# C-H-Chien/Trifocal_Pose_Estimation_using_Improved_GPUHC

Measured on AMD Instinct MI355X. Metric: HC paths/sec (312 tracks x RANSAC samples), higher is better.
Workload: dtype f32

## Files before the change

trifocal_pose_estimation_using_improved_gpuhc_amd/_abi.py:

```python
from __future__ import annotations

import ctypes as C
import os
from collections import namedtuple

import numpy as np

PKG_DIR = os.path.dirname(os.path.abspath(__file__))
LIB_PATH = os.environ.get("HC_TRIFOCAL_LIB") or os.path.join(PKG_DIR, "lib", "libhc_trifocal.so")

ABI_VERSION = 2

NUM_VARS, NUM_PARAMS, NUM_TRACKS = 30, 33, 312
NPP = NUM_PARAMS + 1
UNIFIED_INDEX_SIZE = 38880

HC_STATUS = {0: "HC_SUCCESS", 1: "HC_ERROR_INVALID_VALUE", 2: "HC_ERROR_WORKSPACE", 3: "HC_ERROR_LAUNCH",
             4: "HC_ERROR_DEVICE", 5: "HC_ERROR_TABLE"}


class HCError(RuntimeError):
    pass


# ... 253 lines not shown
P2C_SIGNATURES = (
    Sig("hc_trifocal_2op1p_30x30_track_p2c", _ST, (_TA, C.POINTER(hcP2cArgs), *_WS), True),
    Sig("hc_trifocal_p2c_eval_batched", _ST, (_i, _p, _p, _p, _p, _p, _p, _p, _p, _p, *_WS), True),
    Sig("hc_p2c_coefficients", _ST, (_i, _p, _p, _p, _p, _p), True),
)
P2C_DECLARED_SYMBOLS = tuple(s.name for s in P2C_SIGNATURES)

_RS = C.POINTER(hcRefineSettings)
REFINE_SIGNATURES = (
    Sig("hc_trifocal_pose_refine", _ST, (_p, _i, _p, _p, _RS, _p, _p, _p), True),
    Sig("hc_trifocal_pose_refine_grouped", _ST, (_i, _p, _p, _RS, _p, _p, _p), True),
)
REFINE_DECLARED_SYMBOLS = tuple(s.name for s in REFINE_SIGNATURES)

HC_TOPK_MAX = 32
TOPK_SIGNATURES = (
    Sig("hc_trifocal_pose_topk_joint", _ST, (_i, _p, _p, _i, _p, _p), True),
    Sig("hc_trifocal_pose_topk_joint_grouped", _ST, (_i, _p, _p, _i, _p, _i, _p, _p), True),
    Sig("hc_trifocal_pose_refine_topk", _ST, (_i, _p, _i, _p, _p, _RS, _p, _p, _p, _p, _p), True),
    Sig("hc_trifocal_pose_refine_topk_grouped", _ST, (_i, _p, _i, _p, _RS, _p, _p, _p, _p, _p), True),
    Sig("hc_pose_merge_topk", None, (_i, _i, _p, _p, _p), True),
)
TOPK_DECLARED_SYMBOLS = tuple(s.name for s in TOPK_SIGNATURES)

LU_SIGNATURES = (
    Sig("hc_lu_step_level", _i, (_i,), True),
    Sig("hc_cgesv_30x30_struct_batched", _ST, (_i, _p, _p, _p, _p), True),
    Sig("hc_cgesv_30x30_variant_batched", _ST, (_i, _i, _p, _p, _p, _p), True),
)
LU_VARIANTS = ("throughput", "throughput_twin", "abort", "abort_twin", "small", "small_twin", "archived",
               "archived_twin")
LU_DECLARED_SYMBOLS = tuple(s.name for s in LU_SIGNATURES)

EVAL_SIGNATURES = (
    Sig("hc_trifocal_eval_variant_batched", _ST, (_i, _u, _i, _p, _p, _p, _p, _p, _p, _p, _p, _p, _p, *_WS), True),
)
EVAL_VARIANTS = ("packed", "abs")
HC_EVAL_REDO = 1
EVAL_DECLARED_SYMBOLS = tuple(s.name for s in EVAL_SIGNATURES)

ADAPTIVE_SIGNATURES = (
    Sig("hc_ransac_need_table", _ST, (_i, C.c_double, _i, _i, _p), True),
)
ADAPTIVE_DECLARED_SYMBOLS = tuple(s.name for s in ADAPTIVE_SIGNATURES)

_lib = None


def lib() -> C.CDLL:
    global _lib
    if _lib is None:
        if not os.path.exists(LIB_PATH):
            raise HCError(f"native library missing: {LIB_PATH} (run `python -c 'import __graft_entry__ as g; g.build()'`)")
        import torch
        L = C.CDLL(LIB_PATH)
        for s in SIGNATURES + P2C_SIGNATURES + REFINE_SIGNATURES + TOPK_SIGNATURES + LU_SIGNATURES + \
                EVAL_SIGNATURES + ADAPTIVE_SIGNATURES:
            fn = getattr(L, s.name, None)
            if fn is None:
                if s.optional:
                    continue
                raise HCError(f"{LIB_PATH} does not export {s.name}")
            fn.restype, fn.argtypes = s.restype, list(s.argtypes)
        if L.hc_trifocal_abi_version() != ABI_VERSION:
            raise HCError(f"{LIB_PATH}: ABI {L.hc_trifocal_abi_version()}, this binding expects {ABI_VERSION}")
        _lib = L
    return _lib


def check(status: int, what: str) -> None:
    if status != 0:
        detail = lib().hc_last_error_string().decode(errors="replace")
        raise HCError(f"{what} failed: {HC_STATUS.get(status, status)} ({detail})")


def call(name: str, *args) -> None:
    fn = getattr(lib(), name, None)
    if fn is None:
        raise HCError(f"{LIB_PATH} does not export {name}")
    check(fn(*args), name)


def ptr(x):
    if x is None:
        return C.c_void_p()
    if hasattr(x, "data_ptr"):
        return C.c_void_p(x.data_ptr())
    if hasattr(x, "cuda_stream"):
        return C.c_void_p(x.cuda_stream)
    return x.ctypes.data_as(C.c_void_p)
# ... 35 lines not shown
```

trifocal_pose_estimation_using_improved_gpuhc_amd/csrc/hc_components.hpp:

```cpp
#pragma once

#include "hc_layout.hpp"

namespace hc {


__global__ void __launch_bounds__(WG_THREADS) k_cgesv(int n, const cf *__restrict__ A, const cf *__restrict__ B,
                                                      cf *__restrict__ X) {
    __shared__ LUBuf s_lu[2 * WAVES_PER_WG];
    __shared__ __attribute__((aligned(16))) cf s_scr[2 * WAVES_PER_WG][LU_SCRATCH_CF];
    const int lane = lane_id();
    const int r = lane & 31;
    const int sys = (blockIdx.x * WAVES_PER_WG + threadIdx.x / WAVE) * 2 + (lane >> 5);
    const bool ok = sys < n && r < NV;
    cf rA[NV];
    uint32_t pat = 0;
#pragma unroll
    for (int c = 0; c < NV; c++) {
        rA[c] = ok ? A[((size_t)sys * NV + r) * NV + c] : cmk(0.0f, 0.0f);
        if (rA[c].x != 0.0f || rA[c].y != 0.0f) pat |= 1u << c;
    }
    const cf rB = ok ? B[(size_t)sys * NV + r] : cmk(0.0f, 0.0f);
    LUBuf &LB = s_lu[(threadIdx.x / WAVE) * 2 + (lane >> 5)];
    cf *scr = s_scr[(threadIdx.x / WAVE) * 2 + (lane >> 5)];
    bool redo;
    cf x = lu_solve<false>(rA, rB, lane, pat, LB, scr, redo, __ballot(sys < n));
    if (__builtin_expect(redo, 0)) {
#pragma unroll
        for (int c = 0; c < NV; c++) rA[c] = ok ? A[((size_t)sys * NV + r) * NV + c] : cmk(0.0f, 0.0f);
        x = lu_solve<true>(rA, rB, lane, pat, LB, scr, redo);
    }
    if (ok) X[(size_t)sys * NV + r] = x;
}

__global__ void __launch_bounds__(WG_THREADS) k_cgesv_struct_check(int n, const cf *__restrict__ A,
                                                                   unsigned *__restrict__ bad) {
    const size_t i = (size_t)blockIdx.x * WG_THREADS + threadIdx.x;
    if (i >= (size_t)n * NV) return;
    const uint32_t pat = LU_STRUCT_PAT[i % NV];
    bool out = false;
    for (int c = 0; c < NV; c++) {
        const cf a = A[i * NV + c];
        if (!((pat >> c) & 1u) && (a.x != 0.0f || a.y != 0.0f)) out = true;
    }
    if (out) *bad = 1u;
}
template <int LAT, bool STRUCT, bool ENTCHK, bool FUSE>
__global__ void __launch_bounds__(WG_THREADS) k_cgesv_variant(int n, const cf *__restrict__ A,
                                                              const cf *__restrict__ B, cf *__restrict__ X) {
    __shared__ LUBuf s_lu[2 * WAVES_PER_WG];
    __shared__ __attribute__((aligned(16))) cf s_scr[2 * WAVES_PER_WG][FUSE ? LU_SCRATCH_FUSED_CF : LU_SCRATCH_CF];
    const int lane = lane_id();
    const int r = lane & 31;
    const int sys = (blockIdx.x * WAVES_PER_WG + threadIdx.x / WAVE) * 2 + (lane >> 5);
    const bool ok = sys < n && r < NV;
    cf rA[NV];
    uint32_t nz = 0;
    pf2 sq = {0.0f, 0.0f};
#pragma unroll
    for (int c = 0; c < NV; c++) {
        rA[c] = ok ? A[((size_t)sys * NV + r) * NV + c] : cmk(0.0f, 0.0f);
        if constexpr (!STRUCT) {
            if (rA[c].x != 0.0f || rA[c].y != 0.0f) nz |= 1u << c;
        }
        if constexpr (ENTCHK) {
            sq.x = __builtin_fmaf(rA[c].x, rA[c].x, sq.x);
            sq.y = __builtin_fmaf(rA[c].y, rA[c].y, sq.y);
        }
    }
    bool ent_bad = false;
    if constexpr (ENTCHK) ent_bad = __ballot(!(sq.x + sq.y < __builtin_inff())) != 0ull;
    const uint32_t pat = STRUCT ? (r < NV ? LU_STRUCT_PAT[r] : 0u) : nz;
    const cf rB = ok ? B[(size_t)sys * NV + r] : cmk(0.0f, 0.0f);
    LUBuf &LB = s_lu[(threadIdx.x / WAVE) * 2 + (lane >> 5)];
    cf *scr = s_scr[(threadIdx.x / WAVE) * 2 + (lane >> 5)];
    bool redo;
    cf x = lu_solve<false, LAT, STRUCT, ENTCHK, FUSE>(rA, rB, lane, pat, LB, scr, redo, __ballot(sys < n), ent_bad);
    if (__builtin_expect(redo, 0)) {
#pragma unroll
        for (int c = 0; c < NV; c++) rA[c] = ok ? A[((size_t)sys * NV + r) * NV + c] : cmk(0.0f, 0.0f);
        x = lu_solve<true>(rA, rB, lane, pat, LB, scr, redo);
    }
    if (ok) X[(size_t)sys * NV + r] = x;
}
// ... 165 lines not shown
```

trifocal_pose_estimation_using_improved_gpuhc_amd/csrc/hc_kernels.hip:

```cpp
#include "hc_layout.hpp"
#include "hc_prep.hpp"
#include "hc_components.hpp"
#include "hc_ring.hpp"
#include "hc_score.hpp"
#include "hc_track.hpp"
#include "hc_p2c.hpp"
#include "../../include/hc_trifocal_testing.h"
#include "../../include/p2c/hc_trifocal_p2c.h"
#include "../../include/lu/hc_lu_testing.h"
#include "../../include/eval/hc_eval_testing.h"
#include "../../include/adaptive/hc_trifocal_adaptive.h"

#include <atomic>
#include <climits>
#include <cstdlib>
#include <cstring>
#include <map>
#include <mutex>
#include <utility>

namespace hc {

thread_local hipError_t g_last_hip_error = hipSuccess;
static inline hcStatus launch_status(hcStatus on_fail) {
    const hipError_t e = hipGetLastError();
    if (e != hipSuccess) { g_last_hip_error = e; return on_fail; }
    return HC_SUCCESS;
}

static size_t ws_bytes_needed() { return (sizeof(Workspace) + 255) & ~(size_t)255; }
struct SliceLayout {
    size_t rq, ring, susp;
    size_t total;
    unsigned long long ring_cap;
    size_t susp_entry0, susp_entry1;
};
static SliceLayout slice_layout(long long paths, int max_steps) {
    if (paths < 0) paths = 0;
    if (max_steps < 0) max_steps = 0;
    SliceLayout a;
    a.ring_cap = ring_entries(paths, max_steps);
    const size_t ring_bytes = ((size_t)a.ring_cap * sizeof(unsigned long long) + 255) & ~(size_t)255;
// ... 505 lines not shown
    if ((hc::g_last_hip_error = hipIpcOpenMemHandle(&p, h, hipIpcMemLazyEnablePeerAccess)) != hipSuccess)
        return HC_ERROR_DEVICE;
    *flag = (uint32_t *)p;
    return HC_SUCCESS;
}

hcStatus hc_shared_flag_reset(uint32_t *flag, hcStream stream) {
    if (!flag) return HC_ERROR_INVALID_VALUE;
    if ((hc::g_last_hip_error = hipMemsetAsync(flag, 0, sizeof(uint32_t), (hipStream_t)stream)) != hipSuccess)
        return HC_ERROR_LAUNCH;
    return HC_SUCCESS;
}

hcStatus hc_shared_flag_close(uint32_t *flag, int opened) {
    if (!flag) return HC_ERROR_INVALID_VALUE;
    if (!opened) {
        std::lock_guard<std::mutex> g(hc::g_flag_mu);
        hc::g_flag_kind.erase(flag);
    }
    hc::g_last_hip_error = opened ? hipIpcCloseMemHandle(flag) : hipFree(flag);
    return hc::g_last_hip_error == hipSuccess ? HC_SUCCESS : HC_ERROR_DEVICE;
}

int hc_trifocal_abi_version(void) { return HC_TRIFOCAL_ABI_VERSION; }

unsigned hc_lu_struct_pattern(int row) { return row >= 0 && row < hc::NV ? hc::LU_STRUCT_PAT[row] : 0u; }
unsigned hc_lu_candidates(int step) { return step >= 0 && step < hc::NV ? hc::LU_BOUND.cand[step] : 0u; }
int hc_lu_search_span(int step) { return step >= 0 && step < hc::NV ? hc::lu_search_span(step) : -1; }
int hc_lu_step_level(int step) { return step >= 0 && step < hc::NV ? hc::LU_LEVELS.level[step] : -1; }
int hc_lu_group_class(int step, int group) {
    if (step < 0 || step >= hc::NV - 1 || group < 0 || group >= hc::LuChunks::count(step)) return -1;
    return hc::lu_group_class(step, group);
}

hcStatus hc_trifocal_ring_check_test(void *workspace, size_t workspace_bytes, unsigned head, unsigned tail,
                                     unsigned avail, hcStream stream) {
    const hc::SliceLayout area = hc::slice_layout(0, 0);
    if (!workspace || workspace_bytes < area.ring) return HC_ERROR_WORKSPACE;
    hipStream_t s = (hipStream_t)stream;
    unsigned *rq = (unsigned *)((char *)workspace + area.rq);
    const unsigned v[3] = {head, tail, avail};
    const int at[3] = {hc::RQ_HEAD, hc::RQ_TAIL, hc::RQ_AVAIL};
    (void)hipGetLastError();
    for (int i = 0; i < 3; i++)
        if ((hc::g_last_hip_error = hipMemcpyAsync(rq + at[i], &v[i], sizeof(unsigned), hipMemcpyHostToDevice, s)) !=
            hipSuccess)
            return HC_ERROR_LAUNCH;
    if ((hc::g_last_hip_error = hipStreamSynchronize(s)) != hipSuccess) return HC_ERROR_DEVICE;
    hipLaunchKernelGGL(hc::k_ring_check, dim3(1), dim3(64), 0, s, (hc::Workspace *)workspace, (const unsigned *)rq);
    return hc::launch_status(HC_ERROR_LAUNCH);
}

void hc_trifocal_set_ring_test(int delay_ticks) {
    hc::g_ring_test.store(delay_ticks > 0 ? (delay_ticks < HC_RING_TEST_MIN_TICKS ? HC_RING_TEST_MIN_TICKS : delay_ticks)
                                          : 0,
                          std::memory_order_relaxed);
}

void hc_trifocal_set_small_launch(int mode) {
    hc::g_small_launch.store(mode < 0 ? -1 : mode > 0 ? 1 : 0, std::memory_order_relaxed);
}

void hc_trifocal_set_retry_reuse(int on) { hc::g_retry_reuse.store(on ? 1 : 0, std::memory_order_relaxed); }

const char *hc_trifocal_version(void) {
    return "hc_trifocal gfx950 v10.11 (2 paths/wave, structurally sparse LDS-broadcast LU with lean pivot steps fused by level, "
           "one exec region per pivot step for the eligible rows with the column groups through scratch windows, "
           "column groups by structural class (never-fillable groups untested, always-live groups unconditional), "
           "pivot search narrowed to the candidate rows' DPP group "
           "(abort kernel and tracking launches filling at most half of the path slots -- the latter at 3 waves/SIMD, "
           "16 columns per batch: batched latency mode, one LDS round trip per pivot step, every live-able column "
           "group untested), "
           "structure-agnostic twin kernels for other dH/dx structures, readlane back substitution (the throughput "
           "kernel's fused positions level by level through LDS), pipelined evals over "
           "per-slot prefix tables, 5 waves/SIMD, time slicing at step boundaries with least-attained-service "
           "issue priority, a rejected step's retry reuses its first RK4 slope, the throughput kernel's operand "
           "addresses read complete from per-slot tables and its finiteness check made on the dH/dx entries)";
}

}
```

trifocal_pose_estimation_using_improved_gpuhc_amd/csrc/hc_lu.hpp:

```cpp
#pragma once

#include "hc_eval.hpp"
#include "hc_lu_struct.hpp"
#include "hc_lu_diag.hpp"

namespace hc {

typedef float f4v __attribute__((ext_vector_type(4)));

struct alignas(16) LUBuf {
    cf row[32];
};
static_assert(sizeof(LUBuf) == sizeof(SlotLDS::lu), "LUBuf is SlotLDS::lu");
static_assert(offsetof(SlotLDS, lu) % 16 == 0, "SlotLDS::lu must be 16-B aligned");

__device__ __forceinline__ float rcp_rn(float s) {
    const float r0 = __builtin_amdgcn_rcpf(s);
    const float e0 = __builtin_fmaf(-s, r0, 1.0f);
    return __builtin_fmaf(e0, r0, r0);
}
__device__ __forceinline__ bool rcp_fast_bits(int bits) {
    return (uint32_t)(bits - 0x12800000) < (uint32_t)(0x7B800000 - 0x12800000);
}

// ... 388 lines not shown
            pl1 = 32 + __builtin_ctz((unsigned)(pm >> 32) | 0x80000000u);
            if constexpr (!DENSE)
                redo = redo || __builtin_amdgcn_ballot_w64(!rcp_fast_bits(__float_as_int(piv_abs))) != 0ull;
        } else if constexpr (TIE) {
            const int c2 = key == mx ? rowid : (1 << 20);
            const int mn = half_min_int_p16(c2);
            is_piv = key == mx && rowid == mn;
            piv_abs = __int_as_float(mx);
            const unsigned long long w = __builtin_amdgcn_ballot_w64(is_piv);
            piv_m = w;
            pl0 = __builtin_ctz((unsigned)w);
            pl1 = 32 + __builtin_ctz((unsigned)(w >> 32));
        } else {
            is_piv = __builtin_amdgcn_inverse_ballot_w64(m);
            piv_m = m;
            piv_abs = __int_as_float(mx);
            pl0 = __builtin_ctz(mlo);
            pl1 = 32 + __builtin_ctz(mhi);
        }
        HC_ISA_MARK_I("lu_pattern", I);
        if constexpr (DENSE) lu_step_dense<I>(rA, rB, rowid, my, L, is_piv, reg_s, oo_s, elig HC_LU_WORK_PASS);
        else if constexpr (LAT > 0 && STRUCT) lu_step_batched<I, LAT>(rA, rB, rowid, my, L, scr, is_piv, reg_s, oo_s, elig);
        else lu_step_tested<I, (LAT > 0), STRUCT>(rA, rB, rowid, pat, my, L, scr, is_piv, pl0, pl1, reg_s, oo_s,
                                                  elig HC_LU_WORK_PASS);
        lu_forward<I + 1, DENSE, LAT, STRUCT>(rA, rB, rowid, pat, lane, r, hb, row_lane, my, L, scr, redo,
                                              elig_m & ~piv_m HC_LU_WORK_PASS);
    }
}
template <int LV>
__device__ __forceinline__ void lu_forward_fused(cf (&rA)[NV], cf &rB, int &rowid, uint32_t &pat, int lane, int r, int hb,
                                                 bool row_lane, PivF &my, LUBuf &L, cf *scr, bool &redo,
                                                 unsigned long long elig_m HC_LU_WORK_ARG) {
    if constexpr (LV < LU_LEVELS.nlevels) {
        if (!lu_level<LV>(rA, rB, rowid, pat, lane, r, hb, my, scr, elig_m HC_LU_WORK_PASS)) {
#ifdef HC_DIAG_LUWORK
            lu_work_acc.rare++;
            lu_work_acc.rare_fusable = 1ull;
#endif
            redo = true;
            return;
        }
        lu_forward_fused<LV + 1>(rA, rB, rowid, pat, lane, r, hb, row_lane, my, L, scr, redo, elig_m HC_LU_WORK_PASS);
    } else {
        lu_forward<lu_first_unfused_step(), false, 0, true>(rA, rB, rowid, pat, lane, r, hb, row_lane, my, L, scr, redo,
                                                           elig_m HC_LU_WORK_PASS);
    }
}

template <int I, int LAST = 0>
__device__ __forceinline__ void lu_backward(const cf (&rA)[NV], cf &rB, int rowid, const PivF &my, pf2 &res) {
    if constexpr (I >= LAST) {
        HC_ISA_MARK_I("lu_back", I);
        const unsigned long long own = __builtin_amdgcn_ballot_w64(rowid == I);
        const int o0 = __builtin_ctz((unsigned)own);
        const int o1 = 32 + __builtin_ctz((unsigned)(own >> 32));
        const pf2 q = pcdiv_apply(pf2{rB.x, rB.y}, pf2{rA[I].x, rA[I].y}, my);
        const float x0 = __int_as_float(__builtin_amdgcn_readlane(__float_as_int(q.x), o0));
        const float y0 = __int_as_float(__builtin_amdgcn_readlane(__float_as_int(q.y), o0));
        const float x1 = __int_as_float(__builtin_amdgcn_readlane(__float_as_int(q.x), o1));
        const float y1 = __int_as_float(__builtin_amdgcn_readlane(__float_as_int(q.y), o1));
        const pf2 xs0 = {x0, y0}, xs1 = {x1, y1};
        pf2 xv;
        unsigned long long tmp;
        asm volatile("s_nop 1\n\ts_mov_b64 %2, exec\n\tv_mov_b64 %0, %3\n\ts_mov_b32 exec_lo, 0\n\t"
                     "v_mov_b64 %0, %4\n\ts_mov_b32 exec_lo, %5\n\ts_mov_b32 exec_hi, %5\n\t"
                     "v_mov_b64 %1, %0\n\ts_mov_b64 exec, %2"
                     : "=&v"(xv), "+v"(res), "=&s"(tmp) : "s"(xs0), "s"(xs1), "i"(1u << I));
// ... 10 lines not shown
    const bool entchk = !ABORT && !ARCH && LULAT == 0;
    return LuMode{LULAT, LUS, entchk, entchk && LUS};
}

template <bool DENSE, int LAT = 0, bool STRUCT = false, bool ENTCHK = false, bool FUSE = false>
__device__ __forceinline__ cf lu_solve(cf (&rA)[NV], cf rB, int lane, uint32_t pattern, LUBuf &L, cf *scratch,
                                      bool &redo, unsigned long long count_mask = ~0ull, bool ent_bad = false) {
    static_assert(!FUSE || (!DENSE && LAT == 0 && STRUCT && ENTCHK), "the fused levels belong to the throughput tracker's solve");
    (void)count_mask;
    const int r = lane & 31, hb = lane & 32;
    const bool row_lane = r < NV;
    redo = false;
    if constexpr (DENSE) HC_ISA_MARK("lu_dense");
    else HC_ISA_MARK("lu_sparse");
    HC_ISA_MARK("lu_finite");
    if constexpr (!DENSE && ENTCHK) {
        if (__builtin_expect(ent_bad, 0)) {
            redo = true;
            return cmk(0.0f, 0.0f);
        }
    } else if constexpr (!DENSE) {
        pf2 sq = {0.0f, 0.0f};
#pragma unroll
        for (int c = 0; c < NV; c++) {
            const pf2 e = {rA[c].x, rA[c].y};
            asm("v_pk_fma_f32 %0, %1, %1, %0" : "+v"(sq) : "v"(e));
        }
        const bool ok = sq.x + sq.y < __builtin_inff();
        if (__builtin_expect(__builtin_amdgcn_ballot_w64(!ok) != 0ull, 0)) {
            redo = true;
            return cmk(0.0f, 0.0f);
        }
    }
    int rowid = row_lane ? r : 99;
    uint32_t pat = row_lane ? pattern : 0u;
    PivF my{pf2{0.0f, 0.0f}};
#ifdef HC_DIAG_LUWORK
    LuWork lu_work_acc{0ull, count_mask, 0ull, 0ull, 0ull, 0ull};
#endif
    if constexpr (FUSE)
        lu_forward_fused<0>(rA, rB, rowid, pat, lane, r, hb, row_lane, my, L, scratch + 2 * r, redo,
                            __builtin_amdgcn_ballot_w64(row_lane) HC_LU_WORK_PASS);
    else
        lu_forward<0, DENSE, LAT, STRUCT>(rA, rB, rowid, pat, lane, r, hb, row_lane, my, L, scratch + 2 * r, redo,
                                          __builtin_amdgcn_ballot_w64(row_lane) HC_LU_WORK_PASS);
#ifdef HC_DIAG_LUWORK
    const unsigned long long solves = (unsigned long long)__builtin_popcountll(count_mask & __builtin_amdgcn_ballot_w64(row_lane)) / NV;
    if (lane == 0 && !DENSE && !redo) {
        atomicAdd(&g_diag_luwork[0], lu_work_acc.acc);
        atomicAdd(&g_diag_luwork[1], solves);
        atomicAdd(&g_diag_luwork[3], 1ull);
        atomicAdd(&g_diag_luwork[4], lu_work_acc.groups);
        atomicAdd(&g_diag_luwork[5], lu_work_acc.rare);
    }
    if (lane == 0 && DENSE) atomicAdd(&g_diag_luwork[2], solves);
    if (lane == 0 && !DENSE) atomicAdd(&g_diag_luwork[DIAG_LUWORK_RARE_FUSABLE], lu_work_acc.rare_fusable);
#endif
    if constexpr (FUSE) {
        if (__builtin_expect(redo, 0)) return cmk(0.0f, 0.0f);
    }
#ifdef HC_DIAG_PHASES
    if ((lane & 63) == 0 && blockIdx.x < 16384u) g_diag_lu_mid[blockIdx.x * 4 + (threadIdx.x >> 6)] = __builtin_amdgcn_s_memtime();
#endif
    HC_ISA_MARK("lu_back_init");
    pf2 res = {0.0f, 0.0f};
    if constexpr (FUSE) {
        lu_backward<NV - 1, lu_first_unfused_step()>(rA, rB, rowid, my, res);
// ... 20 lines not shown
```

trifocal_pose_estimation_using_improved_gpuhc_amd/csrc/hc_lu_levels.hpp:

```cpp
#pragma once

namespace hc {

constexpr int DPP_WAVE_SHL1 = 0x130, DPP_WAVE_SHR1 = 0x138;

template <int LV, int K>
__device__ __forceinline__ void lvl_pick(const cf (&rA)[NV], pf2 &c, uint32_t &bnd, int &cwo) {
    if constexpr (K < lu_level_count(LV)) {
        constexpr int I = lu_level_member(LV, K);
        const bool in = __builtin_amdgcn_inverse_ballot_w64(lu_both(LU_BOUND.cand[I]));
        c.x = in ? rA[I].x : c.x;
        c.y = in ? rA[I].y : c.y;
        bnd = in ? LU_BOUND.s[I] : bnd;
        cwo = in ? LU_CHAIN_WIN0 + 2 * K : cwo;
        lvl_pick<LV, K + 1>(rA, c, bnd, cwo);
    }
}
template <int LV, int K>
__device__ __forceinline__ void lvl_relabel(int &rowid, unsigned long long m, int hb) {
    if constexpr (K < lu_level_count(LV)) {
        constexpr int I = lu_level_member(LV, K);
        const unsigned long long mi = and_halves<LU_BOUND.cand[I]>(m);
        const int p0 = __builtin_amdgcn_readlane(rowid, __builtin_ctz((unsigned)mi));
        const int p1 = __builtin_amdgcn_readlane(rowid, 32 + __builtin_ctz((unsigned)(mi >> 32)));
        const int piv_pos = hb ? p1 : p0;
        const bool is_p = __builtin_amdgcn_inverse_ballot_w64(mi);
        rowid = is_p ? I : (rowid == I ? piv_pos : rowid);
        lvl_relabel<LV, K + 1>(rowid, m, hb);
    }
}
template <int LV, int J>
__device__ __forceinline__ void lvl_groups(cf (&rA)[NV], const pf2 &l, cf *wrow, const cf *cw) {
    if constexpr (J < NV) {
        if constexpr (((LU_LEVELS.cols[LV] >> J) & 3u) != 0u) {
            grp_store<J, 2>(wrow, rA);
            wave_lds_sync();
            cf u[2];
            grp_load<J, 2>(cw, u);
            grp_update<J, 2>(rA, l, u);
            __builtin_amdgcn_sched_barrier(0);
        }
        lvl_groups<LV, J + 2>(rA, l, wrow, cw);
    }
}
template <int LV>
__device__ __forceinline__ bool lu_level(cf (&rA)[NV], cf &rB, int &rowid, uint32_t &pat, int lane, int r, int hb,
                                         PivF &my, cf *scr, unsigned long long &elig_m HC_LU_WORK_ARG) {
    constexpr int CNT = lu_level_count(LV), I0 = lu_level_member(LV, 0);
    constexpr uint32_t ROWS = LU_LEVELS.rows[LV];
    HC_ISA_MARK_I("lu_search", I0);
    pf2 c = {0.0f, 0.0f};
    uint32_t bnd = 0u;
    int cwo = 0;
    lvl_pick<LV, 0>(rA, c, bnd, cwo);
    const float v = __builtin_fabsf(c.x) + __builtin_fabsf(c.y);
    pf2 oo_s;
    const pf2 reg_s = recip_fast(c, v, oo_s);
    const unsigned long long lv_elig = and_halves<ROWS>(elig_m);
    const bool elig = __builtin_amdgcn_inverse_ballot_w64(lv_elig);
    const int key = elig ? __float_as_int(v) : -1;
    int mx;
    {
        const int u1 = dpp_i<DPP_WAVE_SHL1>(key), u2 = dpp_i<DPP_WAVE_SHL1>(u1);
        const int d1 = dpp_i<DPP_WAVE_SHR1>(key), d2 = dpp_i<DPP_WAVE_SHR1>(d1);
        const int a = __builtin_amdgcn_inverse_ballot_w64(lu_both(LU_TRI0 | LU_TRI1)) ? u1 : -1;
        const int b = __builtin_amdgcn_inverse_ballot_w64(lu_both(LU_TRI0)) ? u2 : -1;
        const int e = __builtin_amdgcn_inverse_ballot_w64(lu_both(LU_TRI1 | LU_TRI2)) ? d1 : -1;
        const int f = __builtin_amdgcn_inverse_ballot_w64(lu_both(LU_TRI2)) ? d2 : -1;
        mx = max(max(key, a), max(b, max(e, f)));
    }
    constexpr uint32_t UP9 = lu_partner_rows(LV, 9), DN9 = lu_partner_rows(LV, -9), UP6 = lu_partner_rows(LV, 6),
                       DN6 = lu_partner_rows(LV, -6);
    static_assert((UP9 | DN9 | UP6 | DN6 | lu_partner_rows(LV, 0)) == (1u << NV) - 1u, "partner triples 6 or 9 lanes away");
    if constexpr ((UP9 | DN9 | UP6 | DN6) != 0u) {
        int pl = lane;
        if constexpr (UP9 != 0u) pl = __builtin_amdgcn_inverse_ballot_w64(lu_both(UP9)) ? lane + 9 : pl;
        if constexpr (DN9 != 0u) pl = __builtin_amdgcn_inverse_ballot_w64(lu_both(DN9)) ? lane - 9 : pl;
        if constexpr (UP6 != 0u) pl = __builtin_amdgcn_inverse_ballot_w64(lu_both(UP6)) ? lane + 6 : pl;
        if constexpr (DN6 != 0u) pl = __builtin_amdgcn_inverse_ballot_w64(lu_both(DN6)) ? lane - 6 : pl;
        mx = max(mx, __builtin_amdgcn_ds_bpermute(pl << 2, mx));
    }
    const unsigned long long m = and_halves<ROWS>(__builtin_amdgcn_ballot_w64(key == mx));
    const unsigned long long bad = and_halves<ROWS>(__builtin_amdgcn_ballot_w64(!rcp_fast_bits(mx)));
    if (__builtin_expect((__builtin_popcountll(m) != 2 * CNT) | (bad != 0ull), 0)) return false;
    const bool is_piv = __builtin_amdgcn_inverse_ballot_w64(m);
    HC_ISA_MARK_I("lu_store", I0);
    const cf *cw = scr + (cwo - 2 * r);
    cf *wrow = is_piv ? const_cast<cf *>(cw) : scr;
    st4(&wrow[0], cmk(reg_s.x, reg_s.y), rB);
    wave_lds_sync();
    HC_ISA_MARK_I("lu_rcp", I0);
    cf reg, sB0;
    ld4(&cw[0], reg, sB0);
    if (is_piv) my.oo = oo_s;
    asm volatile("" : "+v"(my.oo));
    lvl_relabel<LV, 0>(rowid, m, hb);
    HC_ISA_MARK_I("lu_update", I0);
#ifdef HC_DIAG_LUWORK
    {
        int pairs = 0;
        for (int j = 0; j < NV; j += 2) pairs += ((LU_LEVELS.cols[LV] >> j) & 3u) != 0u;
        lu_work_acc.acc += 2ull * (unsigned long long)pairs *
                           (unsigned long long)__builtin_popcountll(lv_elig & lu_work_acc.mask & ~m);
        lu_work_acc.groups += (unsigned long long)pairs;
    }
#endif
    if (elig) {
        HC_ISA_MARK_I("lu_mult", I0);
        const pf2 lq = pcmul(c, pf2{reg.x, reg.y});
        const pf2 lp = {is_piv ? 0.0f : lq.x, is_piv ? 0.0f : lq.y};
        const pf2 bp = pcmsub(pf2{rB.x, rB.y}, lp, pf2{sB0.x, sB0.y});
        rB = cmk(bp.x, bp.y);
        pat |= (pat & lu_member_cols(LV)) != 0u ? bnd : 0u;
        lvl_groups<LV, 0>(rA, lp, wrow, cw);
    }
    elig_m &= ~m;
    return true;
}

template <int LV, int K>
__device__ __forceinline__ void lvl_back_pick(const cf (&rA)[NV], pf2 &c, int &mem) {
    if constexpr (K < lu_level_count(LV)) {
        constexpr int I = lu_level_member(LV, K);
        if constexpr (K == 0) {
            c = pf2{rA[I].x, rA[I].y};
            mem = I;
        } else {
            const bool in = __builtin_amdgcn_inverse_ballot_w64(lu_both(LU_BOUND.cand[I]));
            c.x = in ? rA[I].x : c.x;
            c.y = in ? rA[I].y : c.y;
            mem = in ? I : mem;
        }
        lvl_back_pick<LV, K + 1>(rA, c, mem);
    }
}
template <int LV>
__device__ __forceinline__ void lu_back_level(const cf (&rA)[NV], cf &rB, int rowid, const PivF &my, LUBuf &L) {
    HC_ISA_MARK_I("lu_back_level", LV);
    pf2 c;
    int mem;
    lvl_back_pick<LV, 0>(rA, c, mem);
    const pf2 q = pcdiv_apply(pf2{rB.x, rB.y}, c, my);
    if (rowid == mem) L.row[mem] = cmk(q.x, q.y);
    wave_lds_sync();
    if constexpr (LV > 0) {
        if (__builtin_amdgcn_inverse_ballot_w64(lu_both(LU_LEVELS.rows[LV]))) {
            const cf x = L.row[mem];
            const pf2 w = pcmsub(pf2{rB.x, rB.y}, pf2{x.x, x.y}, c);
            rB = cmk(w.x, w.y);
        }
    }
}
template <int LV>
__device__ __forceinline__ void lu_backward_fused(const cf (&rA)[NV], cf &rB, int rowid, const PivF &my, LUBuf &L, int r,
                                                  pf2 &res) {
    if constexpr (LV >= 0) {
        lu_back_level<LV>(rA, rB, rowid, my, L);
        lu_backward_fused<LV - 1>(rA, rB, rowid, my, L, r, res);
    } else {
        if (__builtin_amdgcn_inverse_ballot_w64(lu_both(lu_fused_steps()))) {
            const cf x = L.row[r];
            res = pf2{x.x, x.y};
        }
    }
}

}
```

trifocal_pose_estimation_using_improved_gpuhc_amd/csrc/hc_lu_struct.hpp:

```cpp
#pragma once

#include <initializer_list>

#include "hc_device.hpp"

namespace hc {

constexpr int LU_CHUNK = 2;

struct LuChunks {
    static constexpr int single(int I) { return ((I + 1) & 1) && (I + 1 < NV) ? 1 : 0; }
    static constexpr int start(int I, int k) { return k < single(I) ? I + 1 : I + 1 + single(I) + (k - single(I)) * LU_CHUNK; }
    static constexpr int len(int I, int k) {
        return k < single(I) ? 1 : ((NV - start(I, k)) < LU_CHUNK ? (NV - start(I, k)) : LU_CHUNK);
    }
    static constexpr int count(int I) { return single(I) + (NV - (I + 1 + single(I)) + LU_CHUNK - 1) / LU_CHUNK; }
    static constexpr uint32_t mask(int I, int k) { return ((1u << len(I, k)) - 1u) << start(I, k); }
};

constexpr uint32_t LU_STRUCT_PAT[NV] = {
    0x7040004u, 0x7080004u, 0x7100004u, 0x7040009u, 0x7080009u, 0x7100009u, 0x7040012u, 0x7080012u,
    0x7100012u, 0x38200020u, 0x38400020u, 0x38800020u, 0x38200041u, 0x38400041u, 0x38800041u, 0x38200082u,
    0x38400082u, 0x38800082u, 0x7003100u, 0x7003100u, 0x7001100u, 0x7018400u, 0x7018400u, 0x7008400u,
    0x38005200u, 0x38005200u, 0x38001200u, 0x38028800u, 0x38028800u, 0x38008800u};
// ... 149 lines not shown
        if (!((c >> row) & 1u) || lu_popcount(c) <= 3) continue;
        int lo = 0, hi = 31;
        while (!((c >> lo) & 1u)) lo++;
        while (!((c >> hi) & 1u)) hi--;
        return row < lo + 3 ? (hi - 2) - lo : lo - (hi - 2);
    }
    return 0;
}
constexpr uint32_t lu_partner_rows(int lv, int off) {
    uint32_t m = 0u;
    for (int r = 0; r < NV; r++)
        if (lu_partner_off(lv, r) == off) m |= 1u << r;
    return m;
}
constexpr bool lu_chains_are_triples() {
    for (int i = 0; i < NV; i++) {
        if (!lu_step_fusable(i)) continue;
        uint32_t c = LU_BOUND.cand[i], t = 0u;
        for (int q = 0; q < NV; q += 3)
            if (((c >> q) & 7u) == 7u) t |= 7u << q;
        if (t != c) return false;
    }
    return true;
}
static_assert(lu_chains_are_triples(), "a fusable step's candidates are not whole lane triples");
constexpr uint32_t lu_member_cols(int lv) { return LU_LEVELS.fused[lv]; }
constexpr unsigned long long lu_both(uint32_t m) { return (unsigned long long)m | ((unsigned long long)m << 32); }
constexpr uint32_t LU_TRI0 = 0x09249249u, LU_TRI1 = LU_TRI0 << 1, LU_TRI2 = LU_TRI0 << 2;

constexpr int LU_SCRATCH_CF = 2 * 31 + 32;
constexpr int LU_CHAIN_WIN0 = LU_SCRATCH_CF;
constexpr int LU_SCRATCH_FUSED_CF = LU_CHAIN_WIN0 + 2 * (lu_max_level_count() - 1) + 32;

}
```

trifocal_pose_estimation_using_improved_gpuhc_amd/csrc/hc_track_body.inc:

```
    constexpr LuMode LUM = lu_mode(ABORT, ARCH, LULAT, LUS);
    constexpr bool LUSTRUCT = LUM.strct;
    constexpr bool ABSTAB = LUM.entchk;
    constexpr bool LUFUSE = LUM.fuse;
    __shared__ cf s_sp[NPP];
    __shared__ SlotLDS s_slot[2 * WAVES_PER_WG];
    Workspace *ws = a.ws;
    const EvalTables *T = &ws->tab;
    if (ws->status != 0u) return;
    if ((T->lu_struct == 1u) != LUSTRUCT) return;
    const unsigned epoch = (!ABORT && a.slice_q > 0) ? ld_rlx(&a.rq[RQ_EPOCH]) : 0u;
    const uint2 *s_ht = T->ht;
    const uint32_t *s_hx = T->hx;
    const uint32_t *s_hxd = &T->hxd[0][0];
    if (!P2C && threadIdx.x < NPP) s_sp[threadIdx.x] = a.start_params[threadIdx.x];
    {
        float *z = reinterpret_cast<float *>(s_slot);
        for (int i = threadIdx.x; i < (int)(sizeof(s_slot) / 4); i += WG_THREADS) z[i] = 0.0f;
    }
    __syncthreads();
    if (ABORT && threadIdx.x == 0) atomicCAS(&ws->t_start, 0ull, (unsigned long long)__builtin_amdgcn_s_memrealtime());
    const int lane = lane_id();
    const int r = lane & 31, hb = lane & 32;
    const int wid = threadIdx.x / WAVE;
    SlotLDS &S = s_slot[wid * 2 + (hb >> 5)];
    if (r == 30) S.x[30] = cmk(1.0f, 0.0f);
    if (r == 0) S.st.pre_smp = -2;
    __shared__ uint32_t s_rowc[GM_WORDS + 1][32];
    if (threadIdx.x < 32) {
        for (int q = 0; q < GM_WORDS; q++) s_rowc[q][threadIdx.x] = T->gm[q][threadIdx.x];
        s_rowc[GM_WORDS][threadIdx.x] = T->pat[threadIdx.x];
    }
    __syncthreads();
    const bool rl = r < NV;
    wave_lds_sync();
    const AbsTables *AT = &ws->abs;
    const int wv = ABSTAB ? __builtin_amdgcn_readfirstlane(wid) : 0;
    char *const l0 = reinterpret_cast<char *>(s_slot);

    int ph = PH_DEQ, b = -1, smp_loaded = -1;
    int qpos = 0;
    unsigned found_seen = 0u;
#ifdef HC_DIAG_TIMES
    int diag_t0 = 0;
    const unsigned long long diag_w0 = __builtin_amdgcn_s_memrealtime();
    if (lane == 0) atomicMin(&g_diag_span[0], diag_w0);
#endif
    int s = 0, stepidx = 0, coef = 1, succ = 0, nsteps = 0, ncorr = 0;
    int piece = 0;
    float t0 = 0.0f, t_step = 0.0f, dt = 0.01f, h2 = 0.0f, scale = 0.0f;
    bool end_zone = false, check = true, isSucc = false, isInf = false;
    cf x = cmk(0.0f, 0.0f), xl = x, sols = x;
    constexpr bool REUSE = !ABORT && !ARCH;
    bool k1v = false;

#ifdef HC_DIAG_PHASES
    uint64_t dg[8] = {0, 0, 0, 0, 0, 0, 0, 0};
    uint64_t dt_ = __builtin_amdgcn_s_memtime(), dt0_ = dt_;
#define HC_DIAG_MARK(k) do { const uint64_t n_ = __builtin_amdgcn_s_memtime(); dg[k] += n_ - dt_; dt_ = n_; } while (0)
#else
#define HC_DIAG_MARK(k) do { } while (0)
#endif
    for (;;) {
        HC_DIAG_MARK(6);
        HC_ISA_MARK("ctl_slots");
// ... 537 lines not shown
```

Measured before the change: 1.603 million.

## Read fused LU level row constants and row labels from LDS tables

Replaces the per-level chains of compile-time inverse-ballot selects (chain pick, bound, window offset, partner lane, triple-place masks) with a single packed per-row record word loaded from a small LDS table that each workgroup fills at kernel start. Row relabeling after a pivot level now goes through an LDS row-to-position map instead of per-member readlane sequences. The aim is to cut the scalar and VALU instruction count of each fused pivot level. In exchange it adds LDS reads, a table fill with a barrier, a loop in the relabel, and more LDS use that could reduce workgroups per CU.

```diff
diff --git a/include/lu/hc_lu_rowtable_testing.h b/include/lu/hc_lu_rowtable_testing.h
--- /dev/null
+++ b/include/lu/hc_lu_rowtable_testing.h
@@ -0,0 +1,23 @@
+#ifndef HC_LU_ROWTABLE_TESTING_H
+#define HC_LU_ROWTABLE_TESTING_H
+
+#ifdef __cplusplus
+extern "C" {
+#endif
+
+typedef enum {
+    HC_LU_ROW_MEMBER = 0,
+    HC_LU_ROW_BOUND = 1,
+    HC_LU_ROW_WINDOW = 2,
+    HC_LU_ROW_PARTNER = 3,
+    HC_LU_ROW_PLACE = 4,
+    HC_LU_ROW_CHAIN = 5,
+    HC_LU_ROW_FIELD_COUNT = 6
+} hcLuRowField;
+
+int hc_lu_row_field(int level, int row, int field);
+
+#ifdef __cplusplus
+}
+#endif
+#endif
diff --git a/trifocal_pose_estimation_using_improved_gpuhc_amd/_abi.py b/trifocal_pose_estimation_using_improved_gpuhc_amd/_abi.py
--- a/trifocal_pose_estimation_using_improved_gpuhc_amd/_abi.py
+++ b/trifocal_pose_estimation_using_improved_gpuhc_amd/_abi.py
@@ -309,6 +309,11 @@
                "archived_twin")
 LU_DECLARED_SYMBOLS = tuple(s.name for s in LU_SIGNATURES)
 
+LU_ROWTABLE_SIGNATURES = (
+    Sig("hc_lu_row_field", _i, (_i, _i, _i), True),
+)
+LU_ROW_FIELDS = ("member", "bound", "window", "partner", "place", "chain")
+
 EVAL_SIGNATURES = (
     Sig("hc_trifocal_eval_variant_batched", _ST, (_i, _u, _i, _p, _p, _p, _p, _p, _p, _p, _p, _p, _p, *_WS), True),
 )
@@ -332,7 +337,7 @@
         import torch
         L = C.CDLL(LIB_PATH)
         for s in SIGNATURES + P2C_SIGNATURES + REFINE_SIGNATURES + TOPK_SIGNATURES + LU_SIGNATURES + \
-                EVAL_SIGNATURES + ADAPTIVE_SIGNATURES:
+                LU_ROWTABLE_SIGNATURES + EVAL_SIGNATURES + ADAPTIVE_SIGNATURES:
             fn = getattr(L, s.name, None)
             if fn is None:
                 if s.optional:
diff --git a/trifocal_pose_estimation_using_improved_gpuhc_amd/csrc/hc_components.hpp b/trifocal_pose_estimation_using_improved_gpuhc_amd/csrc/hc_components.hpp
--- a/trifocal_pose_estimation_using_improved_gpuhc_amd/csrc/hc_components.hpp
+++ b/trifocal_pose_estimation_using_improved_gpuhc_amd/csrc/hc_components.hpp
@@ -50,6 +50,10 @@
                                                               const cf *__restrict__ B, cf *__restrict__ X) {
     __shared__ LUBuf s_lu[2 * WAVES_PER_WG];
     __shared__ __attribute__((aligned(16))) cf s_scr[2 * WAVES_PER_WG][FUSE ? LU_SCRATCH_FUSED_CF : LU_SCRATCH_CF];
+    if constexpr (FUSE) {
+        lu_rowtab_fill(threadIdx.x);
+        __syncthreads();
+    }
     const int lane = lane_id();
     const int r = lane & 31;
     const int sys = (blockIdx.x * WAVES_PER_WG + threadIdx.x / WAVE) * 2 + (lane >> 5);
diff --git a/trifocal_pose_estimation_using_improved_gpuhc_amd/csrc/hc_kernels.hip b/trifocal_pose_estimation_using_improved_gpuhc_amd/csrc/hc_kernels.hip
--- a/trifocal_pose_estimation_using_improved_gpuhc_amd/csrc/hc_kernels.hip
+++ b/trifocal_pose_estimation_using_improved_gpuhc_amd/csrc/hc_kernels.hip
@@ -8,6 +8,7 @@
 #include "../../include/hc_trifocal_testing.h"
 #include "../../include/p2c/hc_trifocal_p2c.h"
 #include "../../include/lu/hc_lu_testing.h"
+#include "../../include/lu/hc_lu_rowtable_testing.h"
 #include "../../include/eval/hc_eval_testing.h"
 #include "../../include/adaptive/hc_trifocal_adaptive.h"
 
@@ -579,6 +580,21 @@
     if (step < 0 || step >= hc::NV - 1 || group < 0 || group >= hc::LuChunks::count(step)) return -1;
     return hc::lu_group_class(step, group);
 }
+int hc_lu_row_field(int level, int row, int field) {
+    if (level < 0 || level >= hc::LU_REC_LEVELS || row < 0 || row >= hc::LU_REC_ROWS) return -2;
+    hc::LuRowRec rec{0u, hc::LU_ROWTAB.w[level * hc::LU_REC_ROWS + row]};
+    rec.bound = hc::LU_ROWTAB.w[hc::LU_REC_BOUND0 + ((rec.word >> hc::LU_REC_MEMBER_AT) & 31u)];
+    const int mem = (int)((rec.word >> hc::LU_REC_MEMBER_AT) & 31u), k = (int)((rec.word >> hc::LU_REC_CHAIN_AT) & 15u);
+    switch (field) {
+    case HC_LU_ROW_MEMBER: return mem == hc::LU_REC_NO_MEMBER ? -1 : mem;
+    case HC_LU_ROW_BOUND: return (int)rec.bound;
+    case HC_LU_ROW_WINDOW: return (int)(rec.word & ((1u << hc::LU_REC_WIN_BITS) - 1u)) / 8 + 2 * row;
+    case HC_LU_ROW_PARTNER: return (int)((rec.word >> hc::LU_REC_PARTNER_AT) & 31u);
+    case HC_LU_ROW_PLACE: return (rec.word & hc::LU_REC_FIRST) ? 0 : (rec.word & hc::LU_REC_UP) ? 1 : 2;
+    case HC_LU_ROW_CHAIN: return k == hc::LU_REC_NO_CHAIN ? -1 : k;
+    default: return -2;
+    }
+}
 
 hcStatus hc_trifocal_ring_check_test(void *workspace, size_t workspace_bytes, unsigned head, unsigned tail,
                                      unsigned avail, hcStream stream) {
@@ -611,7 +627,7 @@
 void hc_trifocal_set_retry_reuse(int on) { hc::g_retry_reuse.store(on ? 1 : 0, std::memory_order_relaxed); }
 
 const char *hc_trifocal_version(void) {
-    return "hc_trifocal gfx950 v10.11 (2 paths/wave, structurally sparse LDS-broadcast LU with lean pivot steps fused by level, "
+    return "hc_trifocal gfx950 v10.12 (2 paths/wave, structurally sparse LDS-broadcast LU with lean pivot steps fused by level, the levels' per-row constants and row labels read from LDS tables, "
            "one exec region per pivot step for the eligible rows with the column groups through scratch windows, "
            "column groups by structural class (never-fillable groups untested, always-live groups unconditional), "
            "pivot search narrowed to the candidate rows' DPP group "
diff --git a/trifocal_pose_estimation_using_improved_gpuhc_amd/csrc/hc_lu.hpp b/trifocal_pose_estimation_using_improved_gpuhc_amd/csrc/hc_lu.hpp
--- a/trifocal_pose_estimation_using_improved_gpuhc_amd/csrc/hc_lu.hpp
+++ b/trifocal_pose_estimation_using_improved_gpuhc_amd/csrc/hc_lu.hpp
@@ -444,7 +444,7 @@
                                                  bool row_lane, PivF &my, LUBuf &L, cf *scr, bool &redo,
                                                  unsigned long long elig_m HC_LU_WORK_ARG) {
     if constexpr (LV < LU_LEVELS.nlevels) {
-        if (!lu_level<LV>(rA, rB, rowid, pat, lane, r, hb, my, scr, elig_m HC_LU_WORK_PASS)) {
+        if (!lu_level<LV>(rA, rB, rowid, pat, r, hb, my, L, scr, elig_m HC_LU_WORK_PASS)) {
 #ifdef HC_DIAG_LUWORK
             lu_work_acc.rare++;
             lu_work_acc.rare_fusable = 1ull;
@@ -521,7 +521,7 @@
             return cmk(0.0f, 0.0f);
         }
     }
-    int rowid = row_lane ? r : 99;
+    int rowid = row_lane ? r : FUSE ? NV : 99;
     uint32_t pat = row_lane ? pattern : 0u;
     PivF my{pf2{0.0f, 0.0f}};
 #ifdef HC_DIAG_LUWORK
diff --git a/trifocal_pose_estimation_using_improved_gpuhc_amd/csrc/hc_lu_levels.hpp b/trifocal_pose_estimation_using_improved_gpuhc_amd/csrc/hc_lu_levels.hpp
--- a/trifocal_pose_estimation_using_improved_gpuhc_amd/csrc/hc_lu_levels.hpp
+++ b/trifocal_pose_estimation_using_improved_gpuhc_amd/csrc/hc_lu_levels.hpp
@@ -4,30 +4,34 @@
 
 constexpr int DPP_WAVE_SHL1 = 0x130, DPP_WAVE_SHR1 = 0x138;
 
+__device__ __forceinline__ uint32_t *lu_rowtab_lds() {
+    __shared__ uint32_t t[LU_REC_WORDS];
+    return t;
+}
+__device__ __forceinline__ void lu_rowtab_fill(int tid) {
+    if (tid < LU_REC_WORDS) lu_rowtab_lds()[tid] = LU_ROWTAB.w[tid];
+}
 template <int LV, int K>
-__device__ __forceinline__ void lvl_pick(const cf (&rA)[NV], pf2 &c, uint32_t &bnd, int &cwo) {
+__device__ __forceinline__ void lvl_pick(const cf (&rA)[NV], pf2 &c, int kk) {
     if constexpr (K < lu_level_count(LV)) {
         constexpr int I = lu_level_member(LV, K);
-        const bool in = __builtin_amdgcn_inverse_ballot_w64(lu_both(LU_BOUND.cand[I]));
+        const bool in = kk == K;
         c.x = in ? rA[I].x : c.x;
         c.y = in ? rA[I].y : c.y;
-        bnd = in ? LU_BOUND.s[I] : bnd;
-        cwo = in ? LU_CHAIN_WIN0 + 2 * K : cwo;
-        lvl_pick<LV, K + 1>(rA, c, bnd, cwo);
+        lvl_pick<LV, K + 1>(rA, c, kk);
     }
 }
-template <int LV, int K>
-__device__ __forceinline__ void lvl_relabel(int &rowid, unsigned long long m, int hb) {
-    if constexpr (K < lu_level_count(LV)) {
-        constexpr int I = lu_level_member(LV, K);
-        const unsigned long long mi = and_halves<LU_BOUND.cand[I]>(m);
-        const int p0 = __builtin_amdgcn_readlane(rowid, __builtin_ctz((unsigned)mi));
-        const int p1 = __builtin_amdgcn_readlane(rowid, 32 + __builtin_ctz((unsigned)(mi >> 32)));
-        const int piv_pos = hb ? p1 : p0;
-        const bool is_p = __builtin_amdgcn_inverse_ballot_w64(mi);
-        rowid = is_p ? I : (rowid == I ? piv_pos : rowid);
-        lvl_relabel<LV, K + 1>(rowid, m, hb);
+
+template <int LV>
+__device__ __forceinline__ void lvl_relabel(int &rowid, int mem, bool is_piv, unsigned long long live_m, const LUBuf &L) {
+    const bool live = __builtin_amdgcn_inverse_ballot_w64(live_m);
+    for (;;) {
+        const int t = __float_as_int(L.row[rowid].x);
+        rowid = live ? t : rowid;
+        const bool again = live && ((lu_member_cols(LV) >> rowid) & 1u) != 0u;
+        if (__builtin_expect(__builtin_amdgcn_ballot_w64(again) == 0ull, 1)) break;
     }
+    rowid = is_piv ? mem : rowid;
 }
 template <int LV, int J>
 __device__ __forceinline__ void lvl_groups(cf (&rA)[NV], const pf2 &l, cf *wrow, const cf *cw) {
@@ -44,15 +48,14 @@
     }
 }
 template <int LV>
-__device__ __forceinline__ bool lu_level(cf (&rA)[NV], cf &rB, int &rowid, uint32_t &pat, int lane, int r, int hb,
-                                         PivF &my, cf *scr, unsigned long long &elig_m HC_LU_WORK_ARG) {
+__device__ __forceinline__ bool lu_level(cf (&rA)[NV], cf &rB, int &rowid, uint32_t &pat, int r, int hb, PivF &my,
+                                         LUBuf &L, cf *scr, unsigned long long &elig_m HC_LU_WORK_ARG) {
     constexpr int CNT = lu_level_count(LV), I0 = lu_level_member(LV, 0);
     constexpr uint32_t ROWS = LU_LEVELS.rows[LV];
     HC_ISA_MARK_I("lu_search", I0);
     pf2 c = {0.0f, 0.0f};
-    uint32_t bnd = 0u;
-    int cwo = 0;
-    lvl_pick<LV, 0>(rA, c, bnd, cwo);
+    const uint32_t rec = lu_rowtab_lds()[LV * LU_REC_ROWS + r];
+    lvl_pick<LV, 0>(rA, c, (int)((rec >> LU_REC_CHAIN_AT) & 15u));
     const float v = __builtin_fabsf(c.x) + __builtin_fabsf(c.y);
     pf2 oo_s;
     const pf2 reg_s = recip_fast(c, v, oo_s);
@@ -63,21 +66,12 @@
     {
         const int u1 = dpp_i<DPP_WAVE_SHL1>(key), u2 = dpp_i<DPP_WAVE_SHL1>(u1);
         const int d1 = dpp_i<DPP_WAVE_SHR1>(key), d2 = dpp_i<DPP_WAVE_SHR1>(d1);
-        const int a = __builtin_amdgcn_inverse_ballot_w64(lu_both(LU_TRI0 | LU_TRI1)) ? u1 : -1;
-        const int b = __builtin_amdgcn_inverse_ballot_w64(lu_both(LU_TRI0)) ? u2 : -1;
-        const int e = __builtin_amdgcn_inverse_ballot_w64(lu_both(LU_TRI1 | LU_TRI2)) ? d1 : -1;
-        const int f = __builtin_amdgcn_inverse_ballot_w64(lu_both(LU_TRI2)) ? d2 : -1;
-        mx = max(max(key, a), max(b, max(e, f)));
+        const int a = rec >= LU_REC_UP ? u1 : d2;
+        const int b = (int)rec < 0 ? u2 : d1;
+        mx = max(key, max(a, b));
     }
-    constexpr uint32_t UP9 = lu_partner_rows(LV, 9), DN9 = lu_partner_rows(LV, -9), UP6 = lu_partner_rows(LV, 6),
-                       DN6 = lu_partner_rows(LV, -6);
-    static_assert((UP9 | DN9 | UP6 | DN6 | lu_partner_rows(LV, 0)) == (1u << NV) - 1u, "partner triples 6 or 9 lanes away");
-    if constexpr ((UP9 | DN9 | UP6 | DN6) != 0u) {
-        int pl = lane;
-        if constexpr (UP9 != 0u) pl = __builtin_amdgcn_inverse_ballot_w64(lu_both(UP9)) ? lane + 9 : pl;
-        if constexpr (DN9 != 0u) pl = __builtin_amdgcn_inverse_ballot_w64(lu_both(DN9)) ? lane - 9 : pl;
-        if constexpr (UP6 != 0u) pl = __builtin_amdgcn_inverse_ballot_w64(lu_both(UP6)) ? lane + 6 : pl;
-        if constexpr (DN6 != 0u) pl = __builtin_amdgcn_inverse_ballot_w64(lu_both(DN6)) ? lane - 6 : pl;
+    if constexpr (lu_partner_rows(LV, 0) != (1u << NV) - 1u) {
+        const int pl = (int)((rec >> LU_REC_PARTNER_AT) & 31u) + hb;
         mx = max(mx, __builtin_amdgcn_ds_bpermute(pl << 2, mx));
     }
     const unsigned long long m = and_halves<ROWS>(__builtin_amdgcn_ballot_w64(key == mx));
@@ -85,16 +79,20 @@
     if (__builtin_expect((__builtin_popcountll(m) != 2 * CNT) | (bad != 0ull), 0)) return false;
     const bool is_piv = __builtin_amdgcn_inverse_ballot_w64(m);
     HC_ISA_MARK_I("lu_store", I0);
-    const cf *cw = scr + (cwo - 2 * r);
+    const cf *cw = reinterpret_cast<const cf *>(reinterpret_cast<const char *>(scr) + (rec & ((1u << LU_REC_WIN_BITS) - 1u)));
     cf *wrow = is_piv ? const_cast<cf *>(cw) : scr;
     st4(&wrow[0], cmk(reg_s.x, reg_s.y), rB);
+    const int mem = (int)((rec >> LU_REC_MEMBER_AT) & 31u);
+    const uint32_t bnd = lu_rowtab_lds()[LU_REC_BOUND0 + mem];
+    if constexpr (LV == 0) L.row[r].x = __int_as_float(r);
+    if (is_piv) L.row[mem].x = __int_as_float(rowid);
     wave_lds_sync();
     HC_ISA_MARK_I("lu_rcp", I0);
     cf reg, sB0;
     ld4(&cw[0], reg, sB0);
     if (is_piv) my.oo = oo_s;
     asm volatile("" : "+v"(my.oo));
-    lvl_relabel<LV, 0>(rowid, m, hb);
+    lvl_relabel<LV>(rowid, mem, is_piv, elig_m & ~m, L);
     HC_ISA_MARK_I("lu_update", I0);
 #ifdef HC_DIAG_LUWORK
     {
@@ -118,28 +116,13 @@
     return true;
 }
 
-template <int LV, int K>
-__device__ __forceinline__ void lvl_back_pick(const cf (&rA)[NV], pf2 &c, int &mem) {
-    if constexpr (K < lu_level_count(LV)) {
-        constexpr int I = lu_level_member(LV, K);
-        if constexpr (K == 0) {
-            c = pf2{rA[I].x, rA[I].y};
-            mem = I;
-        } else {
-            const bool in = __builtin_amdgcn_inverse_ballot_w64(lu_both(LU_BOUND.cand[I]));
-            c.x = in ? rA[I].x : c.x;
-            c.y = in ? rA[I].y : c.y;
-            mem = in ? I : mem;
-        }
-        lvl_back_pick<LV, K + 1>(rA, c, mem);
-    }
-}
 template <int LV>
-__device__ __forceinline__ void lu_back_level(const cf (&rA)[NV], cf &rB, int rowid, const PivF &my, LUBuf &L) {
+__device__ __forceinline__ void lu_back_level(const cf (&rA)[NV], cf &rB, int rowid, const PivF &my, LUBuf &L, int r) {
     HC_ISA_MARK_I("lu_back_level", LV);
-    pf2 c;
-    int mem;
-    lvl_back_pick<LV, 0>(rA, c, mem);
+    pf2 c = {0.0f, 0.0f};
+    const uint32_t rec = lu_rowtab_lds()[LV * LU_REC_ROWS + r];
+    lvl_pick<LV, 0>(rA, c, (int)((rec >> LU_REC_CHAIN_AT) & 15u));
+    const int mem = (int)((rec >> LU_REC_MEMBER_AT) & 31u);
     const pf2 q = pcdiv_apply(pf2{rB.x, rB.y}, c, my);
     if (rowid == mem) L.row[mem] = cmk(q.x, q.y);
     wave_lds_sync();
@@ -155,7 +138,7 @@
 __device__ __forceinline__ void lu_backward_fused(const cf (&rA)[NV], cf &rB, int rowid, const PivF &my, LUBuf &L, int r,
                                                   pf2 &res) {
     if constexpr (LV >= 0) {
-        lu_back_level<LV>(rA, rB, rowid, my, L);
+        lu_back_level<LV>(rA, rB, rowid, my, L, r);
         lu_backward_fused<LV - 1>(rA, rB, rowid, my, L, r, res);
     } else {
         if (__builtin_amdgcn_inverse_ballot_w64(lu_both(lu_fused_steps()))) {
diff --git a/trifocal_pose_estimation_using_improved_gpuhc_amd/csrc/hc_lu_struct.hpp b/trifocal_pose_estimation_using_improved_gpuhc_amd/csrc/hc_lu_struct.hpp
--- a/trifocal_pose_estimation_using_improved_gpuhc_amd/csrc/hc_lu_struct.hpp
+++ b/trifocal_pose_estimation_using_improved_gpuhc_amd/csrc/hc_lu_struct.hpp
@@ -205,4 +205,53 @@
 constexpr int LU_CHAIN_WIN0 = LU_SCRATCH_CF;
 constexpr int LU_SCRATCH_FUSED_CF = LU_CHAIN_WIN0 + 2 * (lu_max_level_count() - 1) + 32;
 
-}
+struct LuRowRec { uint32_t bound, word; };
+constexpr int LU_REC_WIN_BITS = 10, LU_REC_MEMBER_AT = 10, LU_REC_PARTNER_AT = 15, LU_REC_CHAIN_AT = 20;
+constexpr uint32_t LU_REC_UP = 1u << 30, LU_REC_FIRST = 1u << 31;
+constexpr int LU_REC_NO_MEMBER = 31, LU_REC_NO_CHAIN = 15;
+constexpr int LU_REC_ROWS = 32, LU_REC_LEVELS = 4;
+constexpr int lu_row_chain(int lv, int row) {
+    if (row >= NV) return -1;
+    for (int k = 0; k < lu_level_count(lv); k++)
+        if ((LU_BOUND.cand[lu_level_member(lv, k)] >> row) & 1u) return k;
+    return -1;
+}
+constexpr LuRowRec lu_row_record(int lv, int row) {
+    const int k = lu_row_chain(lv, row);
+    const uint32_t place = (row % 3 == 0 ? LU_REC_FIRST : 0u) | (row % 3 != 2 ? LU_REC_UP : 0u);
+    if (k < 0)
+        return LuRowRec{0u, place | (uint32_t)LU_REC_NO_CHAIN << LU_REC_CHAIN_AT | (uint32_t)row << LU_REC_PARTNER_AT |
+                                (uint32_t)LU_REC_NO_MEMBER << LU_REC_MEMBER_AT};
+    const int I = lu_level_member(lv, k);
+    return LuRowRec{LU_BOUND.s[I], place | (uint32_t)k << LU_REC_CHAIN_AT |
+                                       (uint32_t)(row + lu_partner_off(lv, row)) << LU_REC_PARTNER_AT |
+                                       (uint32_t)I << LU_REC_MEMBER_AT | (uint32_t)(8 * (LU_CHAIN_WIN0 + 2 * k - 2 * row))};
+}
+constexpr int LU_REC_BOUND0 = LU_REC_LEVELS * LU_REC_ROWS, LU_REC_WORDS = LU_REC_BOUND0 + LU_REC_NO_MEMBER + 1;
+struct LuRowTab { uint32_t w[LU_REC_WORDS]; };
+constexpr LuRowTab lu_row_table() {
+    LuRowTab t{};
+    for (int lv = 0; lv < LU_REC_LEVELS; lv++)
+        for (int r = 0; r < LU_REC_ROWS; r++) {
+            const LuRowRec rec = lu_row_record(lv, r);
+            t.w[lv * LU_REC_ROWS + r] = rec.word;
+            t.w[LU_REC_BOUND0 + (int)((rec.word >> LU_REC_MEMBER_AT) & 31u)] = rec.bound;
+        }
+    return t;
+}
+constexpr LuRowTab LU_ROWTAB = lu_row_table();
+constexpr bool lu_row_fields_fit() {
+    for (int lv = 0; lv < LU_REC_LEVELS; lv++)
+        for (int r = 0; r < NV; r++) {
+            const int k = lu_row_chain(lv, r), p = r + lu_partner_off(lv, r);
+            if (k < 0) continue;
+            const int win = 8 * (LU_CHAIN_WIN0 + 2 * k - 2 * r);
+            if (win <= 0 || win >= (1 << LU_REC_WIN_BITS) || k >= LU_REC_NO_CHAIN || p < 0 || p >= NV) return false;
+            if (lu_level_member(lv, k) >= LU_REC_NO_MEMBER || (LU_BOUND.s[lu_level_member(lv, k)] >> NV) != 0u) return false;
+        }
+    return true;
+}
+static_assert(LU_LEVELS.nlevels == LU_REC_LEVELS && lu_row_fields_fit(), "a field of the row records overflows");
+static_assert(LU_REC_WORDS * sizeof(uint32_t) <= 640, "a larger row table may cost the headline kernel its fifth workgroup per CU: measure");
+
+}
diff --git a/trifocal_pose_estimation_using_improved_gpuhc_amd/csrc/hc_track_body.inc b/trifocal_pose_estimation_using_improved_gpuhc_amd/csrc/hc_track_body.inc
--- a/trifocal_pose_estimation_using_improved_gpuhc_amd/csrc/hc_track_body.inc
+++ b/trifocal_pose_estimation_using_improved_gpuhc_amd/csrc/hc_track_body.inc
@@ -30,6 +30,7 @@
         for (int q = 0; q < GM_WORDS; q++) s_rowc[q][threadIdx.x] = T->gm[q][threadIdx.x];
         s_rowc[GM_WORDS][threadIdx.x] = T->pat[threadIdx.x];
     }
+    if constexpr (LUFUSE) lu_rowtab_fill(threadIdx.x);
     __syncthreads();
     const bool rl = r < NV;
     wave_lds_sync();
```

Result: faster. 1.646 million (median of 6 runs) (+2.6%).
